# BichenWuUCB/squeezeDet

Hardware: AMD Instinct MI355X
Metric: images/sec SqueezeDet 1242x375 inference (higher is better)
Workload: dtype f16; 1 GPU; squeezeDet fp16 inference, batch=32 per GPU, synthetic 1242x375 images (4 distinct batches in rotation), full hot path (forward + interpret_output + filter_prediction + filtered rows to pinned host memory), inputs resident in HBM; 2 batches in flight (consecutive steps alternate between 2 HIP streams); global_batch=32, parallelism=dp1 (independent image shards, no collective)

## Files before the change

### include/sqdet.h

```cpp
#ifndef SQDET_H
#define SQDET_H

#include <stddef.h>
#include <stdint.h>

#ifdef __cplusplus
extern "C" {
#endif

typedef void* sqdet_stream_t;

enum { SQDET_OK = 0, SQDET_EINVAL = -1, SQDET_EUNSUPPORTED = -2, SQDET_EHIP = -3, SQDET_ESTATE = -4 };
enum { SQDET_F32 = 0, SQDET_F16 = 1 };
enum { SQDET_PAD_SAME = 0, SQDET_PAD_VALID = 1 };
enum { SQDET_ARCH_SQUEEZEDET = 0, SQDET_ARCH_SQUEEZEDET_PLUS = 1, SQDET_ARCH_RESNET50 = 2, SQDET_ARCH_VGG16 = 3 };

const char* sqdet_version(void);
const char* sqdet_last_error(void);
int sqdet_set_option(const char* name, int value);


size_t sqdet_conv_packed_bytes(int k, int cin, int cout, int dtype);

int sqdet_conv_pack_weights(const float* w_hwio_f32, void* packed, int k, int cin, int cout, int dtype,
// ... 66 lines not shown
                           const void* w_e3, const float* b_e3, void* sq_scratch, void* fire_scratch, void* y,
                           int n, int h, int w, int cin, int s1x1, int e1x1, int e3x3, int dtype, sqdet_stream_t stream);

int sqdet_fire_expand_pair_supported(int n, int h, int w, int s1x1, int e1x1, int e3x3, int dtype);
int sqdet_fire_expand_fwd(const void* sq_in, const void* w_e1, const float* b_e1, const void* w_e3, const float* b_e3,
                          void* y, int n, int h, int w, int s1x1, int e1x1, int e3x3, int pool, int dtype,
                          sqdet_stream_t stream);

int sqdet_fire_squeeze_next_supported(int cin, int s1x1, int e1x1, int e3x3, int next_s1x1, int dtype);
int sqdet_fire_squeeze_next_fwd(const void* x, const void* w_s, const float* b_s, const void* w_e1, const float* b_e1,
                                const void* w_e3, const float* b_e3, const void* w_next_s, const float* b_next_s, void* sq_out,
                                int n, int h, int w, int cin, int s1x1, int e1x1, int e3x3, int next_s1x1, int dtype,
                                sqdet_stream_t stream);

int sqdet_fire_expand_squeeze_next_supported(int s1x1, int e1x1, int e3x3, int next_s1x1, int pool, int dtype);
int sqdet_fire_expand_squeeze_next_fwd(const void* sq_in, const void* w_e1, const float* b_e1, const void* w_e3, const float* b_e3,
                                       const void* w_next_s, const float* b_next_s, void* sq_out, int n, int h, int w, int s1x1,
                                       int e1x1, int e3x3, int next_s1x1, int pool, int dtype, sqdet_stream_t stream);

size_t sqdet_fire_chain_stream_bytes(int s1x1, int e1x1, int e3x3, int next_s1x1, int dtype);
int sqdet_fire_chain_pack(const float* w_e1_hwio, const float* w_e3_hwio, const float* w_next_s_hwio, void* stream_buf,
                          int s1x1, int e1x1, int e3x3, int next_s1x1, int dtype, sqdet_stream_t stream);
int sqdet_fire_chain_fwd(const void* sq_in, const void* stream_buf, const float* b_e1, const float* b_e3,
                         const float* b_next_s, void* y, void* sq_out, int n, int h, int w, int s1x1, int e1x1,
                         int e3x3, int next_s1x1, int dtype, sqdet_stream_t stream);

int sqdet_interpret_output(const void* preds, const float* anchors, float* det_boxes, float* det_probs,
                           int64_t* det_class, float* pred_class_probs, float* pred_conf,
                           int n, int gh, int gw, int apg, int classes, float img_w, float img_h, float exp_thresh,
                           int dtype, sqdet_stream_t stream);
// ... 226 lines not shown
```

### squeezedet_amd/_lib.py

```python
import ctypes as C
import os

_PKG = os.path.dirname(os.path.abspath(__file__))
LIB_PATH = os.environ.get("SQDET_LIB") or os.path.join(_PKG, "libsqdet_hip.so")

SQDET_OK = 0
SQDET_EUNSUPPORTED = -2
F32, F16 = 0, 1
PAD_SAME, PAD_VALID = 0, 1
ARCH_SQUEEZEDET, ARCH_SQUEEZEDET_PLUS, ARCH_RESNET50, ARCH_VGG16 = 0, 1, 2, 3

_lib = None

vp, ci, cf, cd, sz = C.c_void_p, C.c_int, C.c_float, C.c_double, C.c_size_t

SIGNATURES = {
    "sqdet_version": (C.c_char_p, []),
    "sqdet_last_error": (C.c_char_p, []),
    "sqdet_set_option": (ci, [C.c_char_p, ci]),
    "sqdet_conv_packed_bytes": (sz, [ci, ci, ci, ci]),
    "sqdet_conv_pack_weights": (ci, [vp, vp, ci, ci, ci, ci, vp]),
    "sqdet_conv2d_nhwc_fwd": (ci, [vp, vp, vp, vp] + [ci] * 12 + [vp]),
    "sqdet_conv2d_add_nhwc_fwd": (ci, [vp, vp, vp, vp] + [ci] * 12 + [vp]),
    "sqdet_conv2d_res_nhwc_fwd": (ci, [vp, vp, vp, vp, vp] + [ci] * 12 + [vp]),
# ... 9 lines not shown
    "sqdet_maxpool_nhwc_bwd_idx": (ci, [vp, vp, vp, vp] + [ci] * 9 + [vp]),
    "sqdet_conv2d_maxpool2_nhwc_fwd": (ci, [vp, vp, vp, vp] + [ci] * 7 + [vp]),
    "sqdet_conv2d_maxpool2_supported": (ci, [ci] * 6),
    "sqdet_conv2d_maxpool2_nhwc_fwd_idx": (ci, [vp] * 5 + [ci] * 7 + [vp]),
    "sqdet_stem_conv_pool_fwd": (ci, [vp, vp, vp, vp] + [ci] * 8 + [vp]),
    "sqdet_stem_conv_pool_squeeze_supported": (ci, [ci] * 9),
    "sqdet_stem_conv_pool_squeeze_fwd": (ci, [vp] * 6 + [ci] * 9 + [vp]),
    "sqdet_fire_fwd": (ci, [vp] * 9 + [ci] * 8 + [vp]),
    "sqdet_fire_fwd_keep": (ci, [vp] * 9 + [ci] * 8 + [vp]),
    "sqdet_fire_maxpool_fwd": (ci, [vp] * 10 + [ci] * 8 + [vp]),
    "sqdet_fire_expand_fwd": (ci, [vp] * 6 + [ci] * 8 + [vp]),
    "sqdet_fire_expand_pair_supported": (ci, [ci] * 7),
    "sqdet_fire_squeeze_next_supported": (ci, [ci] * 6),
    "sqdet_fire_squeeze_next_fwd": (ci, [vp] * 10 + [ci] * 9 + [vp]),
    "sqdet_fire_expand_squeeze_next_supported": (ci, [ci] * 6),
    "sqdet_fire_expand_squeeze_next_fwd": (ci, [vp] * 8 + [ci] * 9 + [vp]),
    "sqdet_fire_chain_stream_bytes": (sz, [ci] * 5),
    "sqdet_fire_chain_pack": (ci, [vp] * 4 + [ci] * 5 + [vp]),
    "sqdet_fire_chain_fwd": (ci, [vp] * 7 + [ci] * 8 + [vp]),
    "sqdet_interpret_output": (ci, [vp] * 7 + [ci] * 5 + [cf, cf, cf, ci, vp]),
    "sqdet_filter_prediction": (ci, [vp] * 8 + [ci] * 5 + [cd, cf, vp]),
    "sqdet_detect_filter": (ci, [vp] * 8 + [ci] * 5 + [cf, cf, cf, ci, ci, cd, ci, vp]),
    "sqdet_detect_filter_scored": (ci, [vp] * 8 + [ci] * 5 + [cf, cf, cf, ci, ci, cd, ci, ci, vp]),
    "sqdet_net_set_signal": (ci, [vp, ci, vp]),
    "sqdet_net_set_post_job": (ci, [vp] * 9 + [ci] * 5 + [cf, cf, cf, ci, ci, cd, ci]),
    "sqdet_net_rider_capacity": (ci, [vp]),
    "sqdet_net_overlap_layer": (ci, [vp]),
    "sqdet_convdet_fwd": (ci, [vp] * 5 + [ci] * 7 + [vp]),
    "sqdet_convdet_scores_supported": (ci, [ci] * 4),
    "sqdet_net_set_scores": (ci, [vp, vp]),
# ... 147 lines not shown
```

### squeezedet_amd/csrc/fire3.hip

```cpp
#include <type_traits>

#include "conv_common.h"

namespace sqdet {
namespace {

struct FireXArgs {
  const void* sq_in;
  void* s_out;
  const void *w1, *w3, *ws2;
  const float *b1, *b3, *bs2;
  int N, H, W, S, E, S2;
  int tiles_x, tiles_y, ntiles;
  unsigned in_bytes, out_bytes;
  int Hp, Wp, ptp, plp;
};

constexpr int XCOLS = 16;

template <bool S16, bool POOL, int ROWS_T> struct GeoX {
  static constexpr int ROWS = POOL ? 9 : ROWS_T;
  static constexpr int HR = ROWS + 2;
  static constexpr int PXB = S16 ? 32 : 64;
  static constexpr int LW = S16 ? 19 : 24;
  static constexpr int NB = (HR * LW * PXB + 1023) / 1024;
  static constexpr int STILE = NB * 1024;
  static constexpr int RSTEP = POOL ? 8 : ROWS_T, CSTEP = POOL ? 14 : 16;
};

__device__ __forceinline__ void dma16(unsigned voff, const i32x4& rsrc, unsigned lds_dst) {
  asm volatile("s_mov_b32 m0, %2\n\ts_nop 0\n\tbuffer_load_dwordx4 %0, %1, 0 offen lds" ::"v"(voff), "s"(rsrc), "s"(lds_dst) : "memory", "m0");
}
template <int N> __device__ __forceinline__ void vm_wait_x() { asm volatile("s_waitcnt vmcnt(%0)" ::"n"(N) : "memory"); }
__device__ __forceinline__ void lds_barrier() { asm volatile("s_waitcnt lgkmcnt(0)\n\ts_barrier" ::: "memory"); }

__device__ __forceinline__ unsigned int pkmax(unsigned int a, unsigned int b) {
  unsigned int r;
  asm("v_pk_max_f16 %0, %1, %2" : "=v"(r) : "v"(a), "v"(b));
  return r;
}

template <bool S16, bool POOL, int NG, int NTW, int RS, int ROWS_T, int NTS2, int WPS>
__global__ __launch_bounds__((4 * NG / NTW) * RS * 64, WPS) void fire_dma(FireXArgs a) {
  using G = GeoX<S16, POOL, ROWS_T>;
  constexpr int NWAVES = (4 * NG / NTW) * RS;
  constexpr int NT3 = S16 ? 5 : 9;
  constexpr int LW = G::LW, PXB = G::PXB, ROWP = LW * PXB, NB = G::NB, STILE = G::STILE;
  constexpr int NBW = (NB + NWAVES - 1) / NWAVES;
  constexpr int NQ = POOL ? 4 / RS : 0;
  constexpr int MT = POOL ? 2 * NQ + 1 : G::ROWS / RS;
  constexpr int NQC = NG * 4;
  constexpr int CPIX = POOL ? 32 : G::ROWS * 16;
  constexpr int NBLK = CPIX / 16;
  constexpr int NIT = NBLK * NTS2, IPW = (NIT + NWAVES - 1) / NWAVES;
  static_assert(!POOL || RS == 1 || RS == 2, "pooled forms: 4 or 2 pooled rows per wave");
  static_assert(IPW <= 2, "wait counts cover at most two stores per wave and step");
  extern __shared__ __attribute__((aligned(16))) unsigned char lds[];
  unsigned char* sq = lds;
  unsigned char* ctile = sq + 2 * STILE;
  unsigned char* ws2l = ctile + NQC * CPIX * 64;
  float* bl = reinterpret_cast<float*>(ws2l + NQC * NTS2 * 1024);
  const unsigned sq_addr = (unsigned)(uintptr_t)(__attribute__((address_space(3))) unsigned char*)sq;
  const int lane = threadIdx.x & 63;
  const int wave = __builtin_amdgcn_readfirstlane((int)(threadIdx.x >> 6));
  const int j = lane & 15, g = lane >> 4;

  const int xcd = blockIdx.x & 7, lid = blockIdx.x >> 3, nl = gridDim.x >> 3;
  const int per = (a.ntiles + 7) >> 3;
  const int band_end = min(a.ntiles, (xcd + 1) * per);
  int tile = xcd * per + lid;
  if (tile >= band_end) return;

  struct TileXY { int tx, ty, n; };
  auto decode = [&](int t) {
    TileXY c;
    c.tx = t % a.tiles_x; t /= a.tiles_x;
    c.ty = t % a.tiles_y;
    c.n = t / a.tiles_y;
    return c;
  };
  const TileXY dstride = decode(nl);
  auto advance = [&](TileXY& c) {
    c.tx += dstride.tx;
    const int cy = c.tx >= a.tiles_x ? 1 : 0;
    c.tx -= cy ? a.tiles_x : 0;
    c.ty += dstride.ty + cy;
    const int cn = c.ty >= a.tiles_y ? 1 : 0;
    c.ty -= cn ? a.tiles_y : 0;
    c.n += dstride.n + cn;
  };
  TileXY cur = decode(tile), nxt = cur;
  advance(nxt);

  const unsigned long long xaddr = (unsigned long long)(uintptr_t)a.sq_in;
  const i32x4 rin = {(int)(unsigned)xaddr, (int)(unsigned)((xaddr >> 32) & 0xffffu), (int)a.in_bytes, 0x00020000};
  constexpr unsigned OOBL = 0x80000000u;
  unsigned relx[NBW], rcp[NBW];
#pragma unroll
  for (int i = 0; i < NBW; ++i) {
    const int b = wave + NWAVES * i;
    int PL, piece;
    if constexpr (S16) { PL = b * 32 + (lane >> 1); piece = lane & 1; }
    else { PL = b * 16 + (lane >> 2); piece = (lane & 3) ^ ((PL >> 1) & 3); }
    const int r = PL / LW, c = PL - r * LW;
    const bool exists = b < NB && r < G::HR && c < XCOLS + 2;
    relx[i] = exists ? (unsigned)(((r * a.W + c) * a.S + piece * 8) * 2) : OOBL;
    rcp[i] = ((unsigned)r << 16) | (unsigned)c;
  }
  auto issue_dma = [&](const TileXY& tc, int buf) {
    const int hy0 = tc.ty * G::RSTEP - (POOL ? a.ptp : 0) - 1, hx0 = tc.tx * G::CSTEP - (POOL ? a.plp : 0) - 1;
    const bool allin = hy0 >= 0 && hy0 + G::HR <= a.H && hx0 >= 0 && hx0 + XCOLS + 2 <= a.W;
    const unsigned base = (unsigned)((((tc.n * a.H + hy0) * a.W + hx0) * a.S) * 2);
#pragma unroll
    for (int i = 0; i < NBW; ++i) {
      const int b = wave + NWAVES * i;
      if (b < NB) {
        unsigned off = base + relx[i];
        if (!allin) {
          const int iy = hy0 + (int)(rcp[i] >> 16), ix = hx0 + (int)(rcp[i] & 0xffffu);
          if (!(iy >= 0 && iy < a.H && ix >= 0 && ix < a.W)) off = OOBL;
        }
        dma16(off, rin, sq_addr + (unsigned)(buf * STILE + b * 1024));
      }
    }
  };
  issue_dma(cur, 0);

  {
    const i32x4* src2 = reinterpret_cast<const i32x4*>(a.ws2);
    for (int i = threadIdx.x; i < NQC * NTS2 * 64; i += NWAVES * 64) reinterpret_cast<i32x4*>(ws2l)[i] = src2[i];
    for (int i = threadIdx.x; i < 2 * a.E + a.S2; i += NWAVES * 64)
      bl[i] = i < a.E ? a.b1[i] : (i < 2 * a.E ? a.b3[i - a.E] : a.bs2[i - 2 * a.E]);
  }
  const int cw = wave / RS, rq = wave % RS;
  const int cp = NTW == 2 ? cw : cw >> 1;
  const int t0 = NTW == 2 ? 0 : (cw & 1);
  const int m0 = POOL ? rq * 2 * NQ : rq * MT;
  int wsrc[NTW];
#pragma unroll
  for (int t = 0; t < NTW; ++t) {
    const int c = (cp & 1) * 32 + 8 * (j >> 2) + 4 * (t0 + t) + (j & 3);
    wsrc[t] = ((c & 15) >> 2) * 64 + (4 * (c >> 4) + (c & 3)) + 16 * g;
  }
  const int group = cp >> 1;
  i32x4 w3r[NT3][NTW], w1r[NTW];
  {
    const i32x4* p3 = reinterpret_cast<const i32x4*>(a.w3) + (size_t)group * 9 * 4 * 64;
#pragma unroll
    for (int p = 0; p < NT3; ++p) {
#pragma unroll
      for (int t = 0; t < NTW; ++t) {
        if constexpr (S16) {
// ... 5 lines not shown
      }
    }
    const i32x4* p1 = reinterpret_cast<const i32x4*>(a.w1) + (size_t)group * 4 * 64;
#pragma unroll
    for (int t = 0; t < NTW; ++t) w1r[t] = p1[wsrc[t]];
  }
  const int cb = cp * 32 + g * 8 + 4 * t0;

  constexpr int NOFF = S16 ? 6 : 3;
  unsigned boff[NOFF];
  if constexpr (S16) {
#pragma unroll
    for (int p = 0; p < 5; ++p) {
      const int tap = 2 * p + (g >> 1);
      const int dy = tap / 3, dx = tap - dy * 3;
      const int pix = tap < 9 ? (m0 + dy) * LW + j + dx : m0 * LW + XCOLS + 2;
      boff[p] = (unsigned)(pix * PXB + (g & 1) * 16);
    }
    const int pix1 = g < 2 ? (m0 + 1) * LW + j + 1 : m0 * LW + XCOLS + 2;
    boff[5] = (unsigned)(pix1 * PXB + (g & 1) * 16);
  } else {
#pragma unroll
    for (int dx = 0; dx < 3; ++dx) {
      const int P0 = m0 * LW + j + dx;
      boff[dx] = (unsigned)(P0 * 64 + ((g ^ ((P0 >> 1) & 3)) << 4));
    }
  }
  const __amdgpu_buffer_rsrc_t rout = __builtin_amdgcn_make_buffer_rsrc(a.s_out, 0, a.out_bytes, 0x00020000);
  constexpr unsigned OOB = 0xfffffff0u;
  const int nitems = wave < NIT - (IPW - 1) * NWAVES ? IPW : IPW - 1;

  __builtin_amdgcn_s_waitcnt(0x0f70);
  __syncthreads();

  int buf = 0;
  while (true) {
    const bool next_ok = tile + nl < band_end;
    if (next_ok) issue_dma(nxt, buf ^ 1);
    unsigned char* sqb = sq + buf * STILE;
    const int tx = cur.tx, ty = cur.ty, n = cur.n;
    const int oy0 = ty * G::RSTEP - (POOL ? a.ptp : 0), ox0 = tx * G::CSTEP - (POOL ? a.plp : 0);
    const int ox = ox0 + j;
    const bool inside = oy0 + m0 >= 0 && oy0 + m0 + MT <= a.H && ox0 >= 0 && ox0 + XCOLS <= a.W;
    auto conv_pass = [&](auto is3_t, auto ins_t) {
      constexpr bool IS3 = decltype(is3_t)::value;
      constexpr bool INS = decltype(ins_t)::value;
      const float* bias_lds = bl + (IS3 ? a.E : 0) + cb;
      const int chunk = (IS3 ? NQC / 2 : 0) + cp;
      unsigned char* cbase = ctile + chunk * (CPIX * 64) + (NTW == 1 ? t0 * 8 : 0);
      f32x4 run[NTW];
      const float NEGF = __uint_as_float(0xff800000u);
      const bool col_ok = ox >= 0 && ox < a.W;
#pragma unroll
      for (int m = 0; m < MT; ++m) {
        f32x4 acc[NTW];
#pragma unroll
        for (int t = 0; t < NTW; ++t) acc[t] = f32x4{0.f, 0.f, 0.f, 0.f};
        if constexpr (IS3 && S16) {
          i32x4 bf[NT3];
#pragma unroll
          for (int k = 0; k < NT3; ++k) bf[k] = *reinterpret_cast<const i32x4*>(sqb + boff[k] + m * ROWP);
#pragma unroll
          for (int k = 0; k < NT3; ++k)
#pragma unroll
            for (int t = 0; t < NTW; ++t) mma16<f16>(acc[t], w3r[k][t], bf[k]);
        } else if constexpr (IS3) {
#pragma unroll
          for (int dy = 0; dy < 3; ++dy) {
            i32x4 bf[3];
#pragma unroll
            for (int dx = 0; dx < 3; ++dx) bf[dx] = *reinterpret_cast<const i32x4*>(sqb + boff[dx] + (m + dy) * ROWP);
#pragma unroll
            for (int dx = 0; dx < 3; ++dx)
#pragma unroll
              for (int t = 0; t < NTW; ++t) mma16<f16>(acc[t], w3r[dy * 3 + dx][t], bf[dx]);
          }
        } else {
          i32x4 bf1;
          if constexpr (S16) bf1 = *reinterpret_cast<const i32x4*>(sqb + boff[5] + m * ROWP);
          else bf1 = *reinterpret_cast<const i32x4*>(sqb + boff[1] + (m + 1) * ROWP);
#pragma unroll
          for (int t = 0; t < NTW; ++t) mma16<f16>(acc[t], w1r[t], bf1);
        }
        if constexpr (!POOL) {
          unsigned int h[2 * NTW];
#pragma unroll
          for (int t = 0; t < NTW; ++t) {
            f32x4 v = acc[t] + *reinterpret_cast<const f32x4*>(bias_lds + t * 4);
#pragma unroll
            for (int e = 0; e < 4; ++e) v[e] = fmaxf(v[e], 0.f);
            const f16x4 hv = {(f16)v[0], (f16)v[1], (f16)v[2], (f16)v[3]};
            const i32x2 hi = __builtin_bit_cast(i32x2, hv);
            h[2 * t] = (unsigned)hi[0]; h[2 * t + 1] = (unsigned)hi[1];
          }
          const int PLc = (m0 + m) * 16 + j;
          unsigned char* dst = cbase + PLc * 64 + ((g ^ ((PLc >> 1) & 3)) << 4);
          if constexpr (NTW == 2) *reinterpret_cast<i32x4*>(dst) = i32x4{(int)h[0], (int)h[1], (int)h[2], (int)h[3]};
          else *reinterpret_cast<i32x2*>(dst) = i32x2{(int)h[0], (int)h[1]};
        } else {
          if constexpr (!INS) {
            const int oy = oy0 + m0 + m;
            if (!(col_ok && oy >= 0 && oy < a.H)) {
#pragma unroll
              for (int t = 0; t < NTW; ++t) acc[t] = f32x4{NEGF, NEGF, NEGF, NEGF};
            }
          }
          if (m == 0) {
#pragma unroll
            for (int t = 0; t < NTW; ++t) run[t] = acc[t];
          } else {
#pragma unroll
            for (int t = 0; t < NTW; ++t)
#pragma unroll
              for (int e = 0; e < 4; ++e) run[t][e] = __builtin_fmaxf(run[t][e], acc[t][e]);
          }
          if (m >= 2 && (m & 1) == 0) {
            const int q = m / 2 - 1;
            unsigned int vr[2 * NTW];
#pragma unroll
            for (int t = 0; t < NTW; ++t) {
              const f32x4 v = run[t] + *reinterpret_cast<const f32x4*>(bias_lds + t * 4);
              const f16x4 hv = {(f16)v[0], (f16)v[1], (f16)v[2], (f16)v[3]};
              const i32x2 hi = __builtin_bit_cast(i32x2, hv);
              vr[2 * t] = (unsigned)hi[0]; vr[2 * t + 1] = (unsigned)hi[1];
            }
            unsigned int o[2 * NTW];
#pragma unroll
            for (int r = 0; r < 2 * NTW; ++r) {
              const unsigned int s1 = (unsigned int)__builtin_amdgcn_mov_dpp((int)vr[r], 0x101, 0xf, 0xf, true);
              const unsigned int s2 = (unsigned int)__builtin_amdgcn_mov_dpp((int)vr[r], 0x102, 0xf, 0xf, true);
              o[r] = pkmax(pkmax(vr[r], pkmax(s1, s2)), 0u);
            }
            if ((j & 1) == 0 && j <= 12) {
              const int PLc = (rq * NQ + q) * 7 + (j >> 1);
              unsigned char* dst = cbase + PLc * 64 + ((g ^ ((PLc >> 1) & 3)) << 4);
              if constexpr (NTW == 2) *reinterpret_cast<i32x4*>(dst) = i32x4{(int)o[0], (int)o[1], (int)o[2], (int)o[3]};
              else *reinterpret_cast<i32x2*>(dst) = i32x2{(int)o[0], (int)o[1]};
            }
#pragma unroll
            for (int t = 0; t < NTW; ++t) run[t] = acc[t];
          }
        }
      }
    };
    if (!POOL || inside) { conv_pass(std::true_type{}, std::true_type{}); conv_pass(std::false_type{}, std::true_type{}); }
    else { conv_pass(std::true_type{}, std::false_type{}); conv_pass(std::false_type{}, std::false_type{}); }
    lds_barrier();
#pragma unroll
    for (int i = 0; i < IPW; ++i) {
      const int it = wave + NWAVES * i;
      if (it < NIT) {
        const int blk = it / NTS2, t = it - blk * NTS2;
        f32x4 acc2 = f32x4{0.f, 0.f, 0.f, 0.f};
        const int PLc = blk * 16 + j;
        const unsigned char* cb0 = ctile + PLc * 64 + ((g ^ ((PLc >> 1) & 3)) << 4);
        const int cw = 16 * t + j;
        const unsigned char* wb0 = ws2l + ((((cw % (4 * NTS2)) >> 2) * 64 + 4 * (cw / (4 * NTS2)) + (cw & 3) + 16 * g) * 16);
#pragma unroll
        for (int q = 0; q < NQC; ++q)
          mma16<f16>(acc2, *reinterpret_cast<const i32x4*>(wb0 + q * NTS2 * 1024), *reinterpret_cast<const i32x4*>(cb0 + q * (CPIX * 64)));
        int orow, ocol, OH, OW;
        bool ok;
        if constexpr (POOL) {
          const int prow = PLc / 7, pcol = PLc - prow * 7;
          orow = ty * 4 + prow; ocol = tx * 7 + pcol; OH = a.Hp; OW = a.Wp;
          ok = PLc < 28 && orow < OH && ocol < OW;
        } else {
          orow = oy0 + blk; ocol = ox; OH = a.H; OW = a.W;
          ok = orow < OH && ocol < OW;
        }
        const int ch = 16 * t + 4 * g;
        f32x4 v = acc2 + *reinterpret_cast<const f32x4*>(bl + 2 * a.E + ch);
#pragma unroll
        for (int e = 0; e < 4; ++e) v[e] = fmaxf(v[e], 0.f);
        const f16x4 hv = {(f16)v[0], (f16)v[1], (f16)v[2], (f16)v[3]};
        const unsigned off = ok ? (unsigned)((((n * OH + orow) * OW + ocol) * a.S2 + ch) * 2) : OOB;
        __builtin_amdgcn_raw_buffer_store_b64(__builtin_bit_cast(i32x2, hv), rout, off, 0, 0);
      }
    }
    if (!next_ok) break;
    if (nitems == 2) vm_wait_x<2>();
    else if (nitems == 1) vm_wait_x<1>();
    else vm_wait_x<0>();
    lds_barrier();
    tile += nl;
    buf ^= 1;
    cur = nxt;
    advance(nxt);
  }
}

template <bool S16, bool POOL, int NG, int NTW, int RS, int ROWS_T, int NTS2, int WPS>
int launch_dma(const FireXArgs& a, hipStream_t st) {
  using G = GeoX<S16, POOL, ROWS_T>;
  constexpr int NWAVES = (4 * NG / NTW) * RS;
  constexpr int NQC = NG * 4, CPIX = POOL ? 32 : G::ROWS * 16;
  const size_t lds = 2 * (size_t)G::STILE + (size_t)NQC * CPIX * 64 + (size_t)NQC * NTS2 * 1024 + (size_t)(2 * a.E + a.S2) * 4;
  auto kern = &fire_dma<S16, POOL, NG, NTW, RS, ROWS_T, NTS2, WPS>;
  static PerDevice once;
  SQDET_CHECK_HIP(once.run([&] { return hipFuncSetAttribute(reinterpret_cast<const void*>(kern), hipFuncAttributeMaxDynamicSharedMemorySize, 160 * 1024); }));
  constexpr int WGPC = WPS * 4 / NWAVES;
  int grid = cu_count() * WGPC;
  if (grid > (a.ntiles + 7) / 8 * 8) grid = (a.ntiles + 7) / 8 * 8;
  hipLaunchKernelGGL(kern, dim3(grid), dim3(NWAVES * 64), lds, st, a);
  SQDET_CHECK_HIP(hipGetLastError());
  return SQDET_OK;
}

}

int fire_dma_launch(const void* sq_in, const void* w1, const float* b1, const void* w3, const float* b3, const void* ws2,
                    const float* bs2, void* s_out, int n, int h, int w, int s, int e1, int e3, int s2, int pool, int dtype,
                    hipStream_t st, bool* handled) {
  *handled = false;
  const int d = tune(TUNE_DBG);
  if (d == 70 || dtype != SQDET_F16 || e1 != e3) return SQDET_OK;
  const bool f2 = s == 16 && e1 == 64 && s2 == 16 && !pool, f3 = s == 16 && e1 == 64 && s2 == 32 && pool;
  const bool f4 = s == 32 && e1 == 128 && s2 == 32 && !pool, f5 = s == 32 && e1 == 128 && s2 == 48 && pool;
  if (!(f2 || f3 || f4 || f5)) return SQDET_OK;
  FireXArgs a;
  a.sq_in = sq_in; a.s_out = s_out; a.w1 = w1; a.w3 = w3; a.ws2 = ws2; a.b1 = b1; a.b3 = b3; a.bs2 = bs2;
  a.N = n; a.H = h; a.W = w; a.S = s; a.E = e1; a.S2 = s2;
  a.Hp = out_size(h, 3, 2, SQDET_PAD_SAME); a.Wp = out_size(w, 3, 2, SQDET_PAD_SAME);
  a.ptp = pad_before(h, 3, 2, SQDET_PAD_SAME); a.plp = pad_before(w, 3, 2, SQDET_PAD_SAME);
  const int rows_t = (f4 && d != 74 && d != 76 && d != 77) ? 4 : 8;
  if (pool) { a.tiles_x = (a.Wp + 6) / 7; a.tiles_y = (a.Hp + 3) / 4; }
  else { a.tiles_x = (w + XCOLS - 1) / XCOLS; a.tiles_y = (h + rows_t - 1) / rows_t; }
  const long nt = (long)n * a.tiles_x * a.tiles_y;
  const long xb = (long)n * h * w * s * 2, yb = (pool ? (long)n * a.Hp * a.Wp : (long)n * h * w) * s2 * 2;
  if (nt > 0x3fffffffL || xb >= (1L << 31) || yb >= (1L << 31)) return SQDET_OK;
  a.ntiles = (int)nt;
  a.in_bytes = (unsigned)xb; a.out_bytes = (unsigned)yb;
  int rc;
  if (f2) rc = d == 71 ? launch_dma<true, false, 1, 2, 2, 8, 1, 3>(a, st) : launch_dma<true, false, 1, 2, 4, 8, 1, 4>(a, st);
  else if (f3) rc = launch_dma<true, true, 1, 2, 2, 8, 2, 4>(a, st);
  else if (f4) {
    if (d == 74) rc = launch_dma<false, false, 2, 2, 2, 8, 2, 2>(a, st);
    else if (d == 75) rc = launch_dma<false, false, 2, 1, 1, 4, 2, 4>(a, st);
    else if (d == 76) rc = launch_dma<false, false, 2, 2, 4, 8, 2, 4>(a, st);
    else if (d == 77) rc = launch_dma<false, false, 2, 1, 2, 8, 2, 4>(a, st);
    else rc = launch_dma<false, false, 2, 2, 2, 4, 2, 4>(a, st);
// ... 12 lines not shown
```

### squeezedet_amd/csrc/launch.h

```cpp
#pragma once
#include "common.h"

namespace sqdet {

struct ConvArgs;

int conv_algo();
enum { TUNE_C1_WAVES = 0, TUNE_C1_MT = 1, TUNE_C1_MIN_TILES = 2, TUNE_FIRE_FUSE = 3, TUNE_STEM_ALGO = 4, TUNE_DBG = 5, TUNE_G1_WR = 6, TUNE_G1_MBW = 7, TUNE_G1_NTW = 8, TUNE_G1_NS = 9,
       TUNE_CONV_POOL = 10 };
int tune(int which);
int conv2d_launch(const void* x, const void* w_packed, const float* bias, void* y, int n, int h, int w, int cin,
                  int cout, int k, int stride, int pad_mode, int relu, int dtype, int y_cstride, int y_coffset,
                  hipStream_t st);
int conv2d_launch_ex(const void* x, const void* w_packed, const float* bias, void* y, int n, int h, int w, int cin,
                     int cout, int k, int stride, int pad_mode, int relu, int dtype, int y_cstride, int y_coffset,
                     int x_cstride, int x_coffset, int accum, hipStream_t st);
int conv2d_launch_masked(const void* x, const void* w_packed, const float* bias, void* y, int n, int h, int w, int cin,
                         int cout, int k, int stride, int pad_mode, int relu, int dtype, int y_cstride, int y_coffset,
                         int x_cstride, int x_coffset, int accum, const void* relu_of, hipStream_t st);
int convdet_scored_launch(const void* x, const void* w_packed, const float* bias, void* preds, float* scores, int n, int h, int w,
                          int cin, int apg, int classes, int dtype, hipStream_t st);
bool convdet_score_supported(int cout, int apg, int classes, int dtype);

int conv1x1_stream_launch(const ConvArgs& a, const ConvGeom& g, int dtype, hipStream_t st, bool* handled);
// ... 41 lines not shown
                          int pool, hipStream_t st, bool* handled);
bool fire_expand_stream_eligible(int s, int e1, int e3, int dtype);
int fire_expand_stream_launch(const void* sq_in, const void* w1, const float* b1, const void* w3, const float* b3, void* y,
                              int n, int h, int w, int s, int e1, int e3, int dtype, int pool, hipStream_t st, bool* handled);
bool fire_squeeze_next_eligible(int cin, int s, int e1, int e3, int s2, int dtype);
int fire_squeeze_next_launch(const void* x, const void* ws, const float* bs, const void* w1, const float* b1, const void* w3,
                             const float* b3, const void* ws2, const float* bs2, void* s_out, int n, int h, int w, int cin,
                             int s, int e1, int e3, int s2, int dtype, hipStream_t st, bool* handled);
bool fire_expand_squeeze_next_eligible(int s, int e1, int e3, int s2, int pool, int dtype);
int fire_expand_squeeze_next_launch(const void* sq_in, const void* w1, const float* b1, const void* w3, const float* b3,
                                    const void* ws2, const float* bs2, void* s_out, int n, int h, int w, int s, int e1, int e3,
                                    int s2, int pool, int dtype, hipStream_t st, bool* handled);
int fire_dma_launch(const void* sq_in, const void* w1, const float* b1, const void* w3, const float* b3, const void* ws2,
                    const float* bs2, void* s_out, int n, int h, int w, int s, int e1, int e3, int s2, int pool, int dtype,
                    hipStream_t st, bool* handled);

bool fire_chain_eligible(int s, int e1, int e3, int s2, int dtype);

}
```

### squeezedet_amd/csrc/net.cpp

```cpp
#include <math.h>
#include <string.h>

#include <string>
#include <vector>

#include "launch.h"
#include "chain.h"

using namespace sqdet;

namespace {

enum { BUF_INPUT = -1, BUF_PREDS = -2, BUF_A = 0, BUF_B = 1, BUF_S = 2, BUF_T = 3, NUM_BUFS = 4 };
enum { L_CONV = 0, L_POOL = 1, L_STEM = 2, L_FIRE = 3, L_CHAIN = 4, L_EXPAND = 5, L_FIRESQ = 6, L_EXPSQ = 7, L_STEMSQ = 8 };

struct Param {
  std::string name;
  int shape[4];
  int ndim;
  size_t offset;
  size_t bytes;
  int fold = -1;
};

// ... 1013 lines not shown
  const int rc = fire_squeeze_next_launch(x, w_s, b_s, w_e1, b_e1, w_e3, b_e3, w_next_s, b_next_s, sq_out, n, h, w, cin, s1x1, e1x1,
                                          e3x3, next_s1x1, dtype, as_stream(stream), &handled);
  if (rc != SQDET_OK) return rc;
  SQDET_UNSUPPORTED(!handled, "fire_squeeze_next_fwd: shape not covered (see sqdet_fire_squeeze_next_supported)");
  return SQDET_OK;
}

extern "C" int sqdet_fire_squeeze_next_supported(int cin, int s1x1, int e1x1, int e3x3, int next_s1x1, int dtype) {
  return fire_squeeze_next_eligible(cin, s1x1, e1x1, e3x3, next_s1x1, dtype) ? 1 : 0;
}

extern "C" int sqdet_fire_expand_squeeze_next_supported(int s1x1, int e1x1, int e3x3, int next_s1x1, int pool, int dtype) {
  return fire_expand_squeeze_next_eligible(s1x1, e1x1, e3x3, next_s1x1, pool, dtype) ? 1 : 0;
}

extern "C" int sqdet_fire_expand_squeeze_next_fwd(const void* sq_in, const void* w_e1, const float* b_e1, const void* w_e3,
                                                  const float* b_e3, const void* w_next_s, const float* b_next_s, void* sq_out,
                                                  int n, int h, int w, int s1x1, int e1x1, int e3x3, int next_s1x1, int pool,
                                                  int dtype, sqdet_stream_t stream) {
  SQDET_REQUIRE(sq_in && w_e1 && b_e1 && w_e3 && b_e3 && w_next_s && b_next_s && sq_out, "fire_expand_squeeze_next_fwd: null pointer");
  bool handled = false;
  const int rc = fire_expand_squeeze_next_launch(sq_in, w_e1, b_e1, w_e3, b_e3, w_next_s, b_next_s, sq_out, n, h, w, s1x1, e1x1, e3x3,
                                                 next_s1x1, pool, dtype, as_stream(stream), &handled);
  if (rc != SQDET_OK) return rc;
  SQDET_UNSUPPORTED(!handled, "fire_expand_squeeze_next_fwd: shape not covered (see sqdet_fire_expand_squeeze_next_supported)");
  return SQDET_OK;
}
```

Baseline: 84250 images/s.

## Reuse overlapping pooled-row expand results across vertically consecutive fused-fire tiles

The pooled fused expand+squeeze kernel now uses 5-row by 32-column tiles, and each workgroup walks a contiguous run of tiles down a column. The shared boundary row of the 3x3/s2 max-pool is carried in registers from the previous tile, so that row's DMA is skipped and its expand convolution is not recomputed. This cuts redundant halo loads and MMA work, which was much larger under the old 9-row tiles with an 8-row step. In exchange the tile scheduler and carry logic become more complex, and a host-side work-accounting query and a debug grid override are added.

```diff
diff --git a/include/sqdet.h b/include/sqdet.h
--- a/include/sqdet.h
+++ b/include/sqdet.h
@@ -104,6 +104,7 @@
                                 sqdet_stream_t stream);
 
 int sqdet_fire_expand_squeeze_next_supported(int s1x1, int e1x1, int e3x3, int next_s1x1, int pool, int dtype);
+int sqdet_fire_expand_pool_work(int n, int h, int w, int s1x1, int cus, long long* out);
 int sqdet_fire_expand_squeeze_next_fwd(const void* sq_in, const void* w_e1, const float* b_e1, const void* w_e3, const float* b_e3,
                                        const void* w_next_s, const float* b_next_s, void* sq_out, int n, int h, int w, int s1x1,
                                        int e1x1, int e3x3, int next_s1x1, int pool, int dtype, sqdet_stream_t stream);
diff --git a/squeezedet_amd/_lib.py b/squeezedet_amd/_lib.py
--- a/squeezedet_amd/_lib.py
+++ b/squeezedet_amd/_lib.py
@@ -47,6 +47,7 @@
     "sqdet_fire_squeeze_next_supported": (ci, [ci] * 6),
     "sqdet_fire_squeeze_next_fwd": (ci, [vp] * 10 + [ci] * 9 + [vp]),
     "sqdet_fire_expand_squeeze_next_supported": (ci, [ci] * 6),
+    "sqdet_fire_expand_pool_work": (ci, [ci] * 5 + [vp]),
     "sqdet_fire_expand_squeeze_next_fwd": (ci, [vp] * 8 + [ci] * 9 + [vp]),
     "sqdet_fire_chain_stream_bytes": (sz, [ci] * 5),
     "sqdet_fire_chain_pack": (ci, [vp] * 4 + [ci] * 5 + [vp]),
diff --git a/squeezedet_amd/csrc/fire3.hip b/squeezedet_amd/csrc/fire3.hip
--- a/squeezedet_amd/csrc/fire3.hip
+++ b/squeezedet_amd/csrc/fire3.hip
@@ -19,14 +19,36 @@
 constexpr int XCOLS = 16;
 
 template <bool S16, bool POOL, int ROWS_T> struct GeoX {
-  static constexpr int ROWS = POOL ? 9 : ROWS_T;
+  static constexpr int ROWS = POOL ? 5 : ROWS_T;
+  static constexpr int COLS = POOL ? 2 * XCOLS : XCOLS;
   static constexpr int HR = ROWS + 2;
   static constexpr int PXB = S16 ? 32 : 64;
-  static constexpr int LW = S16 ? 19 : 24;
+  static constexpr int LW = S16 ? COLS + 3 : (POOL ? 40 : 24);
   static constexpr int NB = (HR * LW * PXB + 1023) / 1024;
   static constexpr int STILE = NB * 1024;
-  static constexpr int RSTEP = POOL ? 8 : ROWS_T, CSTEP = POOL ? 14 : 16;
+  static constexpr int RSTEP = POOL ? 4 : ROWS_T, CSTEP = POOL ? 30 : 16;
+  static constexpr int PROWS = 2, PCOLS = 15;
 };
+
+struct PoolGeo {
+  int Hp, Wp, ptp, plp, tiles_x, tiles_y;
+};
+inline PoolGeo pool_geo(int h, int w) {
+  PoolGeo p;
+  p.Hp = out_size(h, 3, 2, SQDET_PAD_SAME); p.Wp = out_size(w, 3, 2, SQDET_PAD_SAME);
+  p.ptp = pad_before(h, 3, 2, SQDET_PAD_SAME); p.plp = pad_before(w, 3, 2, SQDET_PAD_SAME);
+  p.tiles_x = (p.Wp + 14) / 15; p.tiles_y = (p.Hp + 1) / 2;
+  return p;
+}
+__host__ __device__ inline void pool_run(int ntiles, int nl, int xcd, int lid, int* first, int* len) {
+  const int per = (ntiles + 7) >> 3;
+  const int band0 = xcd * per;
+  int blen = ntiles - band0;
+  blen = blen > per ? per : (blen < 0 ? 0 : blen);
+  const int base = blen / nl, rem = blen - base * nl;
+  *first = band0 + lid * base + (lid < rem ? lid : rem);
+  *len = base + (lid < rem ? 1 : 0);
+}
 
 __device__ __forceinline__ void dma16(unsigned voff, const i32x4& rsrc, unsigned lds_dst) {
   asm volatile("s_mov_b32 m0, %2\n\ts_nop 0\n\tbuffer_load_dwordx4 %0, %1, 0 offen lds" ::"v"(voff), "s"(rsrc), "s"(lds_dst) : "memory", "m0");
@@ -47,13 +69,13 @@
   constexpr int NT3 = S16 ? 5 : 9;
   constexpr int LW = G::LW, PXB = G::PXB, ROWP = LW * PXB, NB = G::NB, STILE = G::STILE;
   constexpr int NBW = (NB + NWAVES - 1) / NWAVES;
-  constexpr int NQ = POOL ? 4 / RS : 0;
-  constexpr int MT = POOL ? 2 * NQ + 1 : G::ROWS / RS;
+  constexpr int BPW = POOL ? 2 / RS : 1;
+  constexpr int MT = POOL ? G::ROWS : G::ROWS / RS;
   constexpr int NQC = NG * 4;
   constexpr int CPIX = POOL ? 32 : G::ROWS * 16;
   constexpr int NBLK = CPIX / 16;
   constexpr int NIT = NBLK * NTS2, IPW = (NIT + NWAVES - 1) / NWAVES;
-  static_assert(!POOL || RS == 1 || RS == 2, "pooled forms: 4 or 2 pooled rows per wave");
+  static_assert(!POOL || RS == 1 || RS == 2, "pooled forms: two or one column blocks per wave");
   static_assert(IPW <= 2, "wait counts cover at most two stores per wave and step");
   extern __shared__ __attribute__((aligned(16))) unsigned char lds[];
   unsigned char* sq = lds;
@@ -67,27 +89,47 @@
 
   const int xcd = blockIdx.x & 7, lid = blockIdx.x >> 3, nl = gridDim.x >> 3;
   const int per = (a.ntiles + 7) >> 3;
-  const int band_end = min(a.ntiles, (xcd + 1) * per);
-  int tile = xcd * per + lid;
-  if (tile >= band_end) return;
+  int tile = xcd * per + lid, tile_end = min(a.ntiles, (xcd + 1) * per);
+  const int tstep = POOL ? 1 : nl;
+  if constexpr (POOL) {
+    int len;
+    pool_run(a.ntiles, nl, xcd, lid, &tile, &len);
+    tile_end = tile + len;
+  }
+  if (tile >= tile_end) return;
 
   struct TileXY { int tx, ty, n; };
   auto decode = [&](int t) {
     TileXY c;
-    c.tx = t % a.tiles_x; t /= a.tiles_x;
-    c.ty = t % a.tiles_y;
-    c.n = t / a.tiles_y;
+    if constexpr (POOL) {
+      c.ty = t % a.tiles_y; t /= a.tiles_y;
+      c.tx = t % a.tiles_x;
+      c.n = t / a.tiles_x;
+    } else {
+      c.tx = t % a.tiles_x; t /= a.tiles_x;
+      c.ty = t % a.tiles_y;
+      c.n = t / a.tiles_y;
+    }
     return c;
   };
   const TileXY dstride = decode(nl);
   auto advance = [&](TileXY& c) {
-    c.tx += dstride.tx;
-    const int cy = c.tx >= a.tiles_x ? 1 : 0;
-    c.tx -= cy ? a.tiles_x : 0;
-    c.ty += dstride.ty + cy;
-    const int cn = c.ty >= a.tiles_y ? 1 : 0;
-    c.ty -= cn ? a.tiles_y : 0;
-    c.n += dstride.n + cn;
+    if constexpr (POOL) {
+      const int cx = ++c.ty == a.tiles_y ? 1 : 0;
+      c.ty = cx ? 0 : c.ty;
+      c.tx += cx;
+      const int cn = c.tx == a.tiles_x ? 1 : 0;
+      c.tx = cn ? 0 : c.tx;
+      c.n += cn;
+    } else {
+      c.tx += dstride.tx;
+      const int cy = c.tx >= a.tiles_x ? 1 : 0;
+      c.tx -= cy ? a.tiles_x : 0;
+      c.ty += dstride.ty + cy;
+      const int cn = c.ty >= a.tiles_y ? 1 : 0;
+      c.ty -= cn ? a.tiles_y : 0;
+      c.n += dstride.n + cn;
+    }
   };
   TileXY cur = decode(tile), nxt = cur;
   advance(nxt);
@@ -95,7 +137,12 @@
   const unsigned long long xaddr = (unsigned long long)(uintptr_t)a.sq_in;
   const i32x4 rin = {(int)(unsigned)xaddr, (int)(unsigned)((xaddr >> 32) & 0xffffu), (int)a.in_bytes, 0x00020000};
   constexpr unsigned OOBL = 0x80000000u;
-  unsigned relx[NBW], rcp[NBW];
+  unsigned relx[NBW];
+  auto rowcol = [&](int i) {
+    const int PL = (wave + NWAVES * i) * (S16 ? 32 : 16) + (lane >> (S16 ? 1 : 2));
+    const int r = PL / LW;
+    return ((unsigned)r << 16) | (unsigned)(PL - r * LW);
+  };
 #pragma unroll
   for (int i = 0; i < NBW; ++i) {
     const int b = wave + NWAVES * i;
@@ -103,13 +150,12 @@
     if constexpr (S16) { PL = b * 32 + (lane >> 1); piece = lane & 1; }
     else { PL = b * 16 + (lane >> 2); piece = (lane & 3) ^ ((PL >> 1) & 3); }
     const int r = PL / LW, c = PL - r * LW;
-    const bool exists = b < NB && r < G::HR && c < XCOLS + 2;
+    const bool exists = b < NB && r < G::HR && c < G::COLS + 2;
     relx[i] = exists ? (unsigned)(((r * a.W + c) * a.S + piece * 8) * 2) : OOBL;
-    rcp[i] = ((unsigned)r << 16) | (unsigned)c;
-  }
-  auto issue_dma = [&](const TileXY& tc, int buf) {
+  }
+  auto issue_dma = [&](const TileXY& tc, int buf, bool fresh) {
     const int hy0 = tc.ty * G::RSTEP - (POOL ? a.ptp : 0) - 1, hx0 = tc.tx * G::CSTEP - (POOL ? a.plp : 0) - 1;
-    const bool allin = hy0 >= 0 && hy0 + G::HR <= a.H && hx0 >= 0 && hx0 + XCOLS + 2 <= a.W;
+    const bool allin = hy0 + (fresh ? 0 : 1) >= 0 && hy0 + G::HR <= a.H && hx0 >= 0 && hx0 + G::COLS + 2 <= a.W;
     const unsigned base = (unsigned)((((tc.n * a.H + hy0) * a.W + hx0) * a.S) * 2);
 #pragma unroll
     for (int i = 0; i < NBW; ++i) {
@@ -117,14 +163,16 @@
       if (b < NB) {
         unsigned off = base + relx[i];
         if (!allin) {
-          const int iy = hy0 + (int)(rcp[i] >> 16), ix = hx0 + (int)(rcp[i] & 0xffffu);
+          const unsigned rc = rowcol(i);
+          const int iy = hy0 + (int)(rc >> 16), ix = hx0 + (int)(rc & 0xffffu);
           if (!(iy >= 0 && iy < a.H && ix >= 0 && ix < a.W)) off = OOBL;
         }
+        if (POOL && !fresh && rowcol(i) < 0x10000u) off = OOBL;
         dma16(off, rin, sq_addr + (unsigned)(buf * STILE + b * 1024));
       }
     }
   };
-  issue_dma(cur, 0);
+  issue_dma(cur, 0, true);
 
   {
     const i32x4* src2 = reinterpret_cast<const i32x4*>(a.ws2);
@@ -135,7 +183,9 @@
   const int cw = wave / RS, rq = wave % RS;
   const int cp = NTW == 2 ? cw : cw >> 1;
   const int t0 = NTW == 2 ? 0 : (cw & 1);
-  const int m0 = POOL ? rq * 2 * NQ : rq * MT;
+  const int m0 = POOL ? 0 : rq * MT;
+  const int cblk0 = POOL && RS == 2 ? rq : 0;
+  const int jc = j + cblk0 * XCOLS;
   int wsrc[NTW];
 #pragma unroll
   for (int t = 0; t < NTW; ++t) {
@@ -171,15 +221,15 @@
     for (int p = 0; p < 5; ++p) {
       const int tap = 2 * p + (g >> 1);
       const int dy = tap / 3, dx = tap - dy * 3;
-      const int pix = tap < 9 ? (m0 + dy) * LW + j + dx : m0 * LW + XCOLS + 2;
+      const int pix = tap < 9 ? (m0 + dy) * LW + jc + dx : m0 * LW + G::COLS + 2;
       boff[p] = (unsigned)(pix * PXB + (g & 1) * 16);
     }
-    const int pix1 = g < 2 ? (m0 + 1) * LW + j + 1 : m0 * LW + XCOLS + 2;
+    const int pix1 = g < 2 ? (m0 + 1) * LW + jc + 1 : m0 * LW + G::COLS + 2;
     boff[5] = (unsigned)(pix1 * PXB + (g & 1) * 16);
   } else {
 #pragma unroll
     for (int dx = 0; dx < 3; ++dx) {
-      const int P0 = m0 * LW + j + dx;
+      const int P0 = m0 * LW + jc + dx;
       boff[dx] = (unsigned)(P0 * 64 + ((g ^ ((P0 >> 1) & 3)) << 4));
     }
   }
@@ -190,56 +240,61 @@
   __builtin_amdgcn_s_waitcnt(0x0f70);
   __syncthreads();
 
+  auto mac_row = [&](auto is3_t, f32x4 (&acc)[NTW], const unsigned char* sqb, int m, int cbo) {
+    constexpr bool IS3 = decltype(is3_t)::value;
+#pragma unroll
+    for (int t = 0; t < NTW; ++t) acc[t] = f32x4{0.f, 0.f, 0.f, 0.f};
+    if constexpr (IS3 && S16) {
+      i32x4 bf[NT3];
+#pragma unroll
+      for (int k = 0; k < NT3; ++k) {
+        const unsigned bk = k == 2 ? boff[0] + (LW + 1) * PXB : (k == 3 ? boff[0] + 2 * LW * PXB : boff[k]);
+        bf[k] = *reinterpret_cast<const i32x4*>(sqb + bk + m * ROWP + cbo);
+      }
+#pragma unroll
+      for (int k = 0; k < NT3; ++k)
+#pragma unroll
+        for (int t = 0; t < NTW; ++t) mma16<f16>(acc[t], w3r[k][t], bf[k]);
+    } else if constexpr (IS3) {
+#pragma unroll
+      for (int dy = 0; dy < 3; ++dy) {
+        i32x4 bf[3];
+#pragma unroll
+        for (int dx = 0; dx < 3; ++dx) bf[dx] = *reinterpret_cast<const i32x4*>(sqb + boff[dx] + (m + dy) * ROWP + cbo);
+#pragma unroll
+        for (int dx = 0; dx < 3; ++dx)
+#pragma unroll
+          for (int t = 0; t < NTW; ++t) mma16<f16>(acc[t], w3r[dy * 3 + dx][t], bf[dx]);
+      }
+    } else {
+      i32x4 bf1;
+      if constexpr (S16) bf1 = *reinterpret_cast<const i32x4*>(sqb + boff[5] + m * ROWP + cbo);
+      else bf1 = *reinterpret_cast<const i32x4*>(sqb + boff[1] + (m + 1) * ROWP + cbo);
+#pragma unroll
+      for (int t = 0; t < NTW; ++t) mma16<f16>(acc[t], w1r[t], bf1);
+    }
+  };
+  unsigned int car3[BPW][2 * NTW], car1[BPW][2 * NTW];
+  bool fresh = true;
+
   int buf = 0;
   while (true) {
-    const bool next_ok = tile + nl < band_end;
-    if (next_ok) issue_dma(nxt, buf ^ 1);
+    const bool next_ok = tile + tstep < tile_end;
+    if (next_ok) issue_dma(nxt, buf ^ 1, !POOL || nxt.ty == 0);
     unsigned char* sqb = sq + buf * STILE;
     const int tx = cur.tx, ty = cur.ty, n = cur.n;
-    const int oy0 = ty * G::RSTEP - (POOL ? a.ptp : 0), ox0 = tx * G::CSTEP - (POOL ? a.plp : 0);
+    const int oy0 = ty * G::RSTEP - (POOL ? a.ptp : 0), ox0 = tx * G::CSTEP - (POOL ? a.plp : 0) + cblk0 * XCOLS;
     const int ox = ox0 + j;
-    const bool inside = oy0 + m0 >= 0 && oy0 + m0 + MT <= a.H && ox0 >= 0 && ox0 + XCOLS <= a.W;
-    auto conv_pass = [&](auto is3_t, auto ins_t) {
-      constexpr bool IS3 = decltype(is3_t)::value;
-      constexpr bool INS = decltype(ins_t)::value;
-      const float* bias_lds = bl + (IS3 ? a.E : 0) + cb;
-      const int chunk = (IS3 ? NQC / 2 : 0) + cp;
-      unsigned char* cbase = ctile + chunk * (CPIX * 64) + (NTW == 1 ? t0 * 8 : 0);
-      f32x4 run[NTW];
-      const float NEGF = __uint_as_float(0xff800000u);
-      const bool col_ok = ox >= 0 && ox < a.W;
-#pragma unroll
-      for (int m = 0; m < MT; ++m) {
-        f32x4 acc[NTW];
-#pragma unroll
-        for (int t = 0; t < NTW; ++t) acc[t] = f32x4{0.f, 0.f, 0.f, 0.f};
-        if constexpr (IS3 && S16) {
-          i32x4 bf[NT3];
-#pragma unroll
-          for (int k = 0; k < NT3; ++k) bf[k] = *reinterpret_cast<const i32x4*>(sqb + boff[k] + m * ROWP);
-#pragma unroll
-          for (int k = 0; k < NT3; ++k)
-#pragma unroll
-            for (int t = 0; t < NTW; ++t) mma16<f16>(acc[t], w3r[k][t], bf[k]);
-        } else if constexpr (IS3) {
-#pragma unroll
-          for (int dy = 0; dy < 3; ++dy) {
-            i32x4 bf[3];
-#pragma unroll
-            for (int dx = 0; dx < 3; ++dx) bf[dx] = *reinterpret_cast<const i32x4*>(sqb + boff[dx] + (m + dy) * ROWP);
-#pragma unroll
-            for (int dx = 0; dx < 3; ++dx)
-#pragma unroll
-              for (int t = 0; t < NTW; ++t) mma16<f16>(acc[t], w3r[dy * 3 + dx][t], bf[dx]);
-          }
-        } else {
-          i32x4 bf1;
-          if constexpr (S16) bf1 = *reinterpret_cast<const i32x4*>(sqb + boff[5] + m * ROWP);
-          else bf1 = *reinterpret_cast<const i32x4*>(sqb + boff[1] + (m + 1) * ROWP);
-#pragma unroll
-          for (int t = 0; t < NTW; ++t) mma16<f16>(acc[t], w1r[t], bf1);
-        }
-        if constexpr (!POOL) {
+    if constexpr (!POOL) {
+      auto conv_pass = [&](auto is3_t) {
+        constexpr bool IS3 = decltype(is3_t)::value;
+        const float* bias_lds = bl + (IS3 ? a.E : 0) + cb;
+        const int chunk = (IS3 ? NQC / 2 : 0) + cp;
+        unsigned char* cbase = ctile + chunk * (CPIX * 64) + (NTW == 1 ? t0 * 8 : 0);
+#pragma unroll
+        for (int m = 0; m < MT; ++m) {
+          f32x4 acc[NTW];
+          mac_row(is3_t, acc, sqb, m, 0);
           unsigned int h[2 * NTW];
 #pragma unroll
           for (int t = 0; t < NTW; ++t) {
@@ -254,54 +309,107 @@
           unsigned char* dst = cbase + PLc * 64 + ((g ^ ((PLc >> 1) & 3)) << 4);
           if constexpr (NTW == 2) *reinterpret_cast<i32x4*>(dst) = i32x4{(int)h[0], (int)h[1], (int)h[2], (int)h[3]};
           else *reinterpret_cast<i32x2*>(dst) = i32x2{(int)h[0], (int)h[1]};
-        } else {
+        }
+      };
+      conv_pass(std::true_type{});
+      conv_pass(std::false_type{});
+    } else {
+      const int xend = ox0 + BPW * XCOLS;
+      const bool inside = (fresh ? oy0 >= 0 : oy0 + 1 >= 0) && oy0 + MT <= a.H && ox0 >= 0 && xend <= a.W;
+      auto pool_pass = [&](auto is3_t, auto ins_t, unsigned int (&car)[BPW][2 * NTW]) {
+        constexpr bool IS3 = decltype(is3_t)::value;
+        constexpr bool INS = decltype(ins_t)::value;
+        const float* bias_lds = bl + (IS3 ? a.E : 0) + cb;
+        const int chunk = (IS3 ? NQC / 2 : 0) + cp;
+        unsigned char* cbase = ctile + chunk * (CPIX * 64) + (NTW == 1 ? t0 * 8 : 0);
+        const float NEGF = __uint_as_float(0xff800000u);
+        auto put = [&](int PLc, const unsigned int (&o)[2 * NTW]) {
+          unsigned char* dst = cbase + PLc * 64 + ((g ^ ((PLc >> 1) & 3)) << 4);
+          if constexpr (NTW == 2) *reinterpret_cast<i32x4*>(dst) = i32x4{(int)o[0], (int)o[1], (int)o[2], (int)o[3]};
+          else *reinterpret_cast<i32x2*>(dst) = i32x2{(int)o[0], (int)o[1]};
+        };
+#pragma unroll
+        for (int b = 0; b < BPW; ++b) {
+          const int blk = cblk0 + b;
+          const int oxb = ox + b * XCOLS;
           if constexpr (!INS) {
-            const int oy = oy0 + m0 + m;
-            if (!(col_ok && oy >= 0 && oy < a.H)) {
+            if (ox0 + b * XCOLS >= a.W) {
+              if (blk == 1 && j == 0) {
+                const unsigned int z[2 * NTW] = {};
+                put(15, z); put(31, z);
+              }
+              continue;
+            }
+          }
+          const bool col_ok = oxb >= 0 && oxb < a.W;
+          auto row = [&](f32x4 (&acc)[NTW], int m) {
+            bool row_ok = true;
+            if constexpr (!INS) row_ok = oy0 + m >= 0 && oy0 + m < a.H;
+            if (row_ok) {
+              mac_row(is3_t, acc, sqb, m, b * XCOLS * PXB);
+              if constexpr (!INS) {
+                if (!col_ok) {
+#pragma unroll
+                  for (int t = 0; t < NTW; ++t) acc[t] = f32x4{NEGF, NEGF, NEGF, NEGF};
+                }
+              }
+            } else {
 #pragma unroll
               for (int t = 0; t < NTW; ++t) acc[t] = f32x4{NEGF, NEGF, NEGF, NEGF};
             }
-          }
-          if (m == 0) {
-#pragma unroll
-            for (int t = 0; t < NTW; ++t) run[t] = acc[t];
-          } else {
-#pragma unroll
-            for (int t = 0; t < NTW; ++t)
-#pragma unroll
-              for (int e = 0; e < 4; ++e) run[t][e] = __builtin_fmaxf(run[t][e], acc[t][e]);
-          }
-          if (m >= 2 && (m & 1) == 0) {
-            const int q = m / 2 - 1;
-            unsigned int vr[2 * NTW];
+          };
+          auto round16 = [&](const f32x4 (&x)[NTW], unsigned int (&h)[2 * NTW]) {
 #pragma unroll
             for (int t = 0; t < NTW; ++t) {
-              const f32x4 v = run[t] + *reinterpret_cast<const f32x4*>(bias_lds + t * 4);
+              const f32x4 v = x[t] + *reinterpret_cast<const f32x4*>(bias_lds + t * 4);
               const f16x4 hv = {(f16)v[0], (f16)v[1], (f16)v[2], (f16)v[3]};
               const i32x2 hi = __builtin_bit_cast(i32x2, hv);
-              vr[2 * t] = (unsigned)hi[0]; vr[2 * t + 1] = (unsigned)hi[1];
+              h[2 * t] = (unsigned)hi[0]; h[2 * t + 1] = (unsigned)hi[1];
             }
-            unsigned int o[2 * NTW];
-#pragma unroll
-            for (int r = 0; r < 2 * NTW; ++r) {
-              const unsigned int s1 = (unsigned int)__builtin_amdgcn_mov_dpp((int)vr[r], 0x101, 0xf, 0xf, true);
-              const unsigned int s2 = (unsigned int)__builtin_amdgcn_mov_dpp((int)vr[r], 0x102, 0xf, 0xf, true);
-              o[r] = pkmax(pkmax(vr[r], pkmax(s1, s2)), 0u);
+          };
+          f32x4 run[NTW];
+          if (fresh) {
+            row(run, 0);
+            round16(run, car[b]);
+          }
+#pragma unroll
+          for (int m = 1; m < MT; ++m) {
+            f32x4 acc[NTW];
+            row(acc, m);
+            if (m & 1) {
+#pragma unroll
+              for (int t = 0; t < NTW; ++t) run[t] = acc[t];
+            } else {
+#pragma unroll
+              for (int t = 0; t < NTW; ++t)
+#pragma unroll
+                for (int e = 0; e < 4; ++e) run[t][e] = __builtin_fmaxf(run[t][e], acc[t][e]);
+              const int q = m / 2 - 1;
+              unsigned int vr[2 * NTW];
+              round16(run, vr);
+#pragma unroll
+              for (int r = 0; r < 2 * NTW; ++r) vr[r] = pkmax(vr[r], car[b][r]);
+              round16(acc, car[b]);
+              unsigned int o[2 * NTW];
+#pragma unroll
+              for (int r = 0; r < 2 * NTW; ++r) {
+                const unsigned int s1 = (unsigned int)__builtin_amdgcn_mov_dpp((int)vr[r], 0x101, 0xf, 0xf, true);
+                const unsigned int s2 = (unsigned int)__builtin_amdgcn_mov_dpp((int)vr[r], 0x102, 0xf, 0xf, true);
+                o[r] = pkmax(pkmax(vr[r], pkmax(s1, s2)), 0u);
+              }
+              if ((j & 1) == 0 && j <= (blk == 0 ? 14 : 12)) put(q * 16 + blk * 8 + (j >> 1), o);
+              if (blk == 1 && j == 0) {
+#pragma unroll
+                for (int r = 0; r < 2 * NTW; ++r) o[r] = pkmax(vr[r], 0u);
+                put(q * 16 + 15, o);
+              }
             }
-            if ((j & 1) == 0 && j <= 12) {
-              const int PLc = (rq * NQ + q) * 7 + (j >> 1);
-              unsigned char* dst = cbase + PLc * 64 + ((g ^ ((PLc >> 1) & 3)) << 4);
-              if constexpr (NTW == 2) *reinterpret_cast<i32x4*>(dst) = i32x4{(int)o[0], (int)o[1], (int)o[2], (int)o[3]};
-              else *reinterpret_cast<i32x2*>(dst) = i32x2{(int)o[0], (int)o[1]};
-            }
-#pragma unroll
-            for (int t = 0; t < NTW; ++t) run[t] = acc[t];
           }
         }
-      }
-    };
-    if (!POOL || inside) { conv_pass(std::true_type{}, std::true_type{}); conv_pass(std::false_type{}, std::true_type{}); }
-    else { conv_pass(std::true_type{}, std::false_type{}); conv_pass(std::false_type{}, std::false_type{}); }
+      };
+      if (inside) { pool_pass(std::true_type{}, std::true_type{}, car3); pool_pass(std::false_type{}, std::true_type{}, car1); }
+      else { pool_pass(std::true_type{}, std::false_type{}, car3); pool_pass(std::false_type{}, std::false_type{}, car1); }
+    }
     lds_barrier();
 #pragma unroll
     for (int i = 0; i < IPW; ++i) {
@@ -311,17 +419,24 @@
         f32x4 acc2 = f32x4{0.f, 0.f, 0.f, 0.f};
         const int PLc = blk * 16 + j;
         const unsigned char* cb0 = ctile + PLc * 64 + ((g ^ ((PLc >> 1) & 3)) << 4);
+        const unsigned char* cf0 = POOL && j == 7 ? cb0 + 8 * 64 : cb0;
         const int cw = 16 * t + j;
         const unsigned char* wb0 = ws2l + ((((cw % (4 * NTS2)) >> 2) * 64 + 4 * (cw / (4 * NTS2)) + (cw & 3) + 16 * g) * 16);
 #pragma unroll
-        for (int q = 0; q < NQC; ++q)
-          mma16<f16>(acc2, *reinterpret_cast<const i32x4*>(wb0 + q * NTS2 * 1024), *reinterpret_cast<const i32x4*>(cb0 + q * (CPIX * 64)));
+        for (int q = 0; q < NQC; ++q) {
+          i32x4 bq = *reinterpret_cast<const i32x4*>(cb0 + q * (CPIX * 64));
+          if constexpr (POOL) {
+            const i32x4 fq = *reinterpret_cast<const i32x4*>(cf0 + q * (CPIX * 64));
+#pragma unroll
+            for (int e = 0; e < 4; ++e) bq[e] = (int)pkmax((unsigned)bq[e], (unsigned)fq[e]);
+          }
+          mma16<f16>(acc2, *reinterpret_cast<const i32x4*>(wb0 + q * NTS2 * 1024), bq);
+        }
         int orow, ocol, OH, OW;
         bool ok;
         if constexpr (POOL) {
-          const int prow = PLc / 7, pcol = PLc - prow * 7;
-          orow = ty * 4 + prow; ocol = tx * 7 + pcol; OH = a.Hp; OW = a.Wp;
-          ok = PLc < 28 && orow < OH && ocol < OW;
+          orow = ty * G::PROWS + blk; ocol = tx * G::PCOLS + j; OH = a.Hp; OW = a.Wp;
+          ok = j < G::PCOLS && orow < OH && ocol < OW;
         } else {
           orow = oy0 + blk; ocol = ox; OH = a.H; OW = a.W;
           ok = orow < OH && ocol < OW;
@@ -340,8 +455,9 @@
     else if (nitems == 1) vm_wait_x<1>();
     else vm_wait_x<0>();
     lds_barrier();
-    tile += nl;
+    tile += tstep;
     buf ^= 1;
+    fresh = POOL && nxt.ty == 0;
     cur = nxt;
     advance(nxt);
   }
@@ -358,12 +474,50 @@
   SQDET_CHECK_HIP(once.run([&] { return hipFuncSetAttribute(reinterpret_cast<const void*>(kern), hipFuncAttributeMaxDynamicSharedMemorySize, 160 * 1024); }));
   constexpr int WGPC = WPS * 4 / NWAVES;
   int grid = cu_count() * WGPC;
+  if (POOL && tune(TUNE_DBG) == 72) grid = 8;
   if (grid > (a.ntiles + 7) / 8 * 8) grid = (a.ntiles + 7) / 8 * 8;
   hipLaunchKernelGGL(kern, dim3(grid), dim3(NWAVES * 64), lds, st, a);
   SQDET_CHECK_HIP(hipGetLastError());
   return SQDET_OK;
 }
 
+}
+
+int fire_dma_pool_work(int n, int h, int w, int s, int cus, long long* out) {
+  if (n < 1 || h < 1 || w < 1 || cus < 1 || (s != 16 && s != 32)) return SQDET_EINVAL;
+  const PoolGeo pg = pool_geo(h, w);
+  const long nt = (long)n * pg.tiles_x * pg.tiles_y;
+  if (nt > 0x3fffffffL) return SQDET_EINVAL;
+  const int wgpc = s == 16 ? 4 : 2;
+  int grid = cus * wgpc;
+  if (grid > (nt + 7) / 8 * 8) grid = (int)((nt + 7) / 8 * 8);
+  const int nl = grid >> 3;
+  long long eval = 0, pooled = 0;
+  long next = 0;
+  bool ordered = nl > 0;
+  for (int xcd = 0; xcd < 8 && nl > 0; ++xcd)
+    for (int lid = 0; lid < nl; ++lid) {
+      int first, len;
+      pool_run((int)nt, nl, xcd, lid, &first, &len);
+      if (len == 0) continue;
+      ordered = ordered && first == next;
+      next = first + len;
+      for (int t = first; t < first + len; ++t) {
+        const int ty = t % pg.tiles_y, tx = (t / pg.tiles_y) % pg.tiles_x;
+        const bool fresh = t == first || ty == 0;
+        const int oy0 = ty * 4 - pg.ptp, ox0 = tx * 30 - pg.plp;
+        int rows = 0, blocks = 0;
+        for (int m = fresh ? 0 : 1; m < 5; ++m) rows += oy0 + m >= 0 && oy0 + m < h;
+        for (int b = 0; b < 2; ++b) blocks += ox0 + 16 * b < w;
+        eval += rows * blocks;
+        const int pr = pg.Hp - 2 * ty, pc = pg.Wp - 15 * tx;
+        pooled += (pr < 2 ? pr : 2) * (pc < 15 ? pc : 15);
+      }
+    }
+  out[0] = eval; out[1] = (long long)n * (((long long)h * w + 15) / 16);
+  out[2] = pooled; out[3] = (long long)n * pg.Hp * pg.Wp;
+  out[4] = ordered && next == nt ? 1 : 0;
+  return SQDET_OK;
 }
 
 int fire_dma_launch(const void* sq_in, const void* w1, const float* b1, const void* w3, const float* b3, const void* ws2,
@@ -381,7 +535,7 @@
   a.Hp = out_size(h, 3, 2, SQDET_PAD_SAME); a.Wp = out_size(w, 3, 2, SQDET_PAD_SAME);
   a.ptp = pad_before(h, 3, 2, SQDET_PAD_SAME); a.plp = pad_before(w, 3, 2, SQDET_PAD_SAME);
   const int rows_t = (f4 && d != 74 && d != 76 && d != 77) ? 4 : 8;
-  if (pool) { a.tiles_x = (a.Wp + 6) / 7; a.tiles_y = (a.Hp + 3) / 4; }
+  if (pool) { const PoolGeo pg = pool_geo(h, w); a.tiles_x = pg.tiles_x; a.tiles_y = pg.tiles_y; }
   else { a.tiles_x = (w + XCOLS - 1) / XCOLS; a.tiles_y = (h + rows_t - 1) / rows_t; }
   const long nt = (long)n * a.tiles_x * a.tiles_y;
   const long xb = (long)n * h * w * s * 2, yb = (pool ? (long)n * a.Hp * a.Wp : (long)n * h * w) * s2 * 2;
diff --git a/squeezedet_amd/csrc/launch.h b/squeezedet_amd/csrc/launch.h
--- a/squeezedet_amd/csrc/launch.h
+++ b/squeezedet_amd/csrc/launch.h
@@ -79,6 +79,7 @@
 int fire_dma_launch(const void* sq_in, const void* w1, const float* b1, const void* w3, const float* b3, const void* ws2,
                     const float* bs2, void* s_out, int n, int h, int w, int s, int e1, int e3, int s2, int pool, int dtype,
                     hipStream_t st, bool* handled);
+int fire_dma_pool_work(int n, int h, int w, int s, int cus, long long* out);
 
 bool fire_chain_eligible(int s, int e1, int e3, int s2, int dtype);
 
diff --git a/squeezedet_amd/csrc/net.cpp b/squeezedet_amd/csrc/net.cpp
--- a/squeezedet_amd/csrc/net.cpp
+++ b/squeezedet_amd/csrc/net.cpp
@@ -1051,6 +1051,11 @@
   return fire_expand_squeeze_next_eligible(s1x1, e1x1, e3x3, next_s1x1, pool, dtype) ? 1 : 0;
 }
 
+extern "C" int sqdet_fire_expand_pool_work(int n, int h, int w, int s1x1, int cus, long long* out) {
+  SQDET_REQUIRE(out, "fire_expand_pool_work: null pointer");
+  return fire_dma_pool_work(n, h, w, s1x1, cus, out);
+}
+
 extern "C" int sqdet_fire_expand_squeeze_next_fwd(const void* sq_in, const void* w_e1, const float* b_e1, const void* w_e3,
                                                   const float* b_e3, const void* w_next_s, const float* b_next_s, void* sq_out,
                                                   int n, int h, int w, int s1x1, int e1x1, int e3x3, int next_s1x1, int pool,
```

Result: slower. 82380 images/s (-2.2%).
